# google-research/simclr

Hardware: AMD Instinct MI355X
Metric: images/sec (whole node), ResNet-50 1x SimCLR pretraining step @224px (higher is better)
Workload: dtype f32; 1 GPU; ResNet-50 1x, 224x224, 2 views/image, per-GPU batch 512, global batch 512, NT-Xent T=0.1 + linear-eval head + LARS, global BN, dp1; global_batch=512, parallelism=dp1

## Files before the change

simclr_amd/csrc/conv.hip:

```cpp
#include "common.h"
#include <stdlib.h>
#include <string.h>
#include <mutex>
#include <type_traits>

namespace {

enum { MODE_FWD = 0, MODE_DGRAD = 1 };

struct ConvP {
  const void* x;
  const void* w;
  void* y;
  float* stats;
  int V, IH, IW, IC, OH, OW, N, KH, KW, stride, pad;
  int pixpitch;
  int M, K;
  int nslot, accumulate;
  int m_tiles, n_tiles;
  int cs, py, px, cls_h, cls_w;
  int ntaps;
  int taps[9];
  unsigned long long tap_w, dy_w, dx_w;
  const void* bn_x;
// ... 1919 lines not shown
    const unsigned char* ds = xs + p.hpp * RB;
#pragma unroll
    for (int ks = 0; ks < 2; ++ks) {
      u32x4 bf[4];
#pragma unroll
      for (int ni = 0; ni < 4; ++ni) {
        const s16x4_t lo = __builtin_amdgcn_ds_read_tr16_b64_v4i16((lds_s16x4_t*)(ds + ks * 32 * RB + b_lo[ni]));
        const s16x4_t hi = __builtin_amdgcn_ds_read_tr16_b64_v4i16((lds_s16x4_t*)(ds + ks * 32 * RB + b_hi[ni]));
        const u32x2 l2 = __builtin_bit_cast(u32x2, lo), h2 = __builtin_bit_cast(u32x2, hi);
        bf[ni] = (u32x4){l2[0], l2[1], h2[0], h2[1]};
      }
      const int jw = p.W - gx[ks];
      const unsigned lowm = jw >= 8 ? 0xffu : ((1u << jw) - 1u);
      const int y1 = (gy[ks] + 1 == p.H) ? 0 : gy[ks] + 1;
      const unsigned up = (gy[ks] > 0 ? lowm : 0u) | (y1 > 0 ? (0xffu & ~lowm) : 0u);
      const unsigned dn = (gy[ks] < p.H - 1 ? lowm : 0u) | (y1 < p.H - 1 ? (0xffu & ~lowm) : 0u);
      const unsigned lf = 0xffu & ~((gx[ks] == 0 ? 1u : 0u) | (jw < 8 ? (1u << jw) : 0u));
      const unsigned rt = 0xffu & ~((jw - 1 < 8 ? (1u << (jw - 1)) : 0u) |
                                    (jw - 1 + p.W < 8 ? (1u << (jw - 1 + p.W)) : 0u));
      u32x4 wup, wdn, wlf, wrt;
#pragma unroll
      for (int d = 0; d < 4; ++d) {
        wup[d] = (((up >> (2 * d)) & 1u) ? 0x0000ffffu : 0u) | (((up >> (2 * d + 1)) & 1u) ? 0xffff0000u : 0u);
        wdn[d] = (((dn >> (2 * d)) & 1u) ? 0x0000ffffu : 0u) | (((dn >> (2 * d + 1)) & 1u) ? 0xffff0000u : 0u);
        wlf[d] = (((lf >> (2 * d)) & 1u) ? 0x0000ffffu : 0u) | (((lf >> (2 * d + 1)) & 1u) ? 0xffff0000u : 0u);
        wrt[d] = (((rt >> (2 * d)) & 1u) ? 0x0000ffffu : 0u) | (((rt >> (2 * d + 1)) & 1u) ? 0xffff0000u : 0u);
      }
#pragma unroll
      for (int t = 0; t < 9; ++t) {
        const int ty = t / 3, tx = t % 3;
        const s16x4_t lo = __builtin_amdgcn_ds_read_tr16_b64_v4i16((lds_s16x4_t*)(xs + ks * 32 * RB + a_lo[t]));
        const s16x4_t hi = __builtin_amdgcn_ds_read_tr16_b64_v4i16((lds_s16x4_t*)(xs + ks * 32 * RB + a_hi[t]));
        const u32x2 l2 = __builtin_bit_cast(u32x2, lo), h2 = __builtin_bit_cast(u32x2, hi);
        u32x4 af = (u32x4){l2[0], l2[1], h2[0], h2[1]};
        if (t != 4) {
#pragma unroll
          for (int d = 0; d < 4; ++d) {
            unsigned w = 0xffffffffu;
            if (ty == 0) w &= wup[d]; else if (ty == 2) w &= wdn[d];
            if (tx == 0) w &= wlf[d]; else if (tx == 2) w &= wrt[d];
            af[d] &= w;
          }
        }
#pragma unroll
        for (int ni = 0; ni < 4; ++ni)
          acc[t][ni] = __builtin_amdgcn_mfma_f32_16x16x32_bf16(
              __builtin_bit_cast(bf16x8, bf[ni]), __builtin_bit_cast(bf16x8, af), acc[t][ni], 0, 0, 0);
      }
      gx[ks] += dcol;
      if (gx[ks] >= p.W) { gx[ks] -= p.W; ++gy[ks]; }
      gy[ks] += drow;
      if (gy[ks] >= p.H) gy[ks] -= p.H;
    }
  };

  int issued = c_begin, cs = 0, is = ST - 1;
#pragma unroll
  for (int s = 0; s < ST - 1; ++s)
    if (issued < c_end) { issue(issued, s); ++issued; }
  const int nq = p.hpp >> 5;
  for (int c = c_begin; c < c_end; ++c) {
    if (ST == 3 && issued - c - 1 >= 1 && nq == 3) asm volatile("s_waitcnt vmcnt(5)" ::: "memory");
    else if (ST == 3 && issued - c - 1 >= 1 && nq == 4) asm volatile("s_waitcnt vmcnt(6)" ::: "memory");
    else asm volatile("s_waitcnt vmcnt(0)" ::: "memory");
    __syncthreads();
    if (issued < c_end) { issue(issued, is); ++issued; is = (is + 1 == ST) ? 0 : is + 1; }
    compute(cs);
    cs = (cs + 1 == ST) ? 0 : cs + 1;
  }
  float* slab = p.dw + (long long)split * 9 * p.IC * p.N;
#pragma unroll
  for (int t = 0; t < 9; ++t) {
    const int kk = t * p.IC + ci0 + wave * 16 + fl;
#pragma unroll
    for (int ni = 0; ni < 4; ++ni) {
      const int n = n0 + ni * 16 + g * 4;
      *(float4*)(slab + (long long)kk * p.N + n) = make_float4(acc[t][ni][0], acc[t][ni][1], acc[t][ni][2], acc[t][ni][3]);
    }
  }
}

__device__ __forceinline__ int w3f_key(int row) { return (row & 3) | (((row >> 3) & 1) << 2); }

__global__ __launch_bounds__(256, 2) void conv_wgrad3x3_f32ps(const Wgrad3P p) {
  constexpr int BR = 32, RB = 256;
  extern __shared__ __attribute__((aligned(16))) unsigned char smem[];
  typedef __attribute__((address_space(1))) const void* gptr_t;
  typedef __attribute__((address_space(3))) void* lptr_t;
  const int tid = threadIdx.x, lane = tid & 63;
  const int wave = __builtin_amdgcn_readfirstlane(tid >> 6);
  const int g = lane >> 4, fl = lane & 15;
  const int tiles = p.ci_tiles * p.co_tiles;
  const int xcd = blockIdx.x & 7, bidx = blockIdx.x >> 3;
  const int tile = bidx % tiles, split = (bidx / tiles) * 8 + xcd;
  if (split >= p.splits) return;
  const int ci0 = (tile % p.ci_tiles) * 64, n0 = (tile / p.ci_tiles) * 64;
  const float* __restrict__ X = (const float*)p.x;
  const float* __restrict__ DY = (const float*)p.dy;
  const int W1 = p.W + 1;
  const int stage_bytes = (p.hpp + BR) * RB;

  f32x4 acc[9][4];
#pragma unroll
  for (int t = 0; t < 9; ++t)
#pragma unroll
    for (int j = 0; j < 4; ++j) acc[t][j] = (f32x4){0.f, 0.f, 0.f, 0.f};

  const int nchunks = (p.M + BR - 1) / BR;
  const int c_begin = split * p.chunks_per_split;
  const int c_end = min(nchunks, c_begin + p.chunks_per_split);

  const int lrow = lane >> 4, lpc = lane & 15;
  auto issue = [&](int c, int s) __attribute__((always_inline)) {
    unsigned char* xs = smem + s * stage_bytes;
    unsigned char* ds = xs + p.hpp * RB;
    const int mc = c * BR;
    const int nxi = p.hpp >> 2;
    for (int q = wave; q < nxi; q += 4) {
      const int r = q * 4 + lrow;
      const int lc = (((lpc >> 1) ^ w3f_key(r)) << 1) | (lpc & 1);
      const int gp = mc + r - W1;
      const void* src = (gp >= 0 && gp < p.M) ? (const void*)(X + (long long)gp * p.pixpitch + ci0 + lc * 4) : p.zero;
      __builtin_amdgcn_global_load_lds((gptr_t)src, (lptr_t)(xs + q * 1024), 16, 0, 0);
    }
#pragma unroll
    for (int j = 0; j < 2; ++j) {
      const int q = wave * 2 + j;
      const int r = q * 4 + lrow;
      const int lc = (((lpc >> 1) ^ w3f_key(r)) << 1) | (lpc & 1);
      const int m = mc + r;
      const void* src = (m < p.M) ? (const void*)(DY + (long long)m * p.N + n0 + lc * 4) : p.zero;
      __builtin_amdgcn_global_load_lds((gptr_t)src, (lptr_t)(ds + q * 1024), 16, 0, 0);
    }
  };

  auto off_of = [&](int row, int byte) -> int { return row * RB + (((byte >> 5) ^ w3f_key(row)) << 5) + (byte & 31); };
  const int px_lane = g * 8 + (fl >> 2);
  const int xbyte = (wave >> 1) * 128 + (wave & 1) * 32 + (fl & 3) * 8;
  auto hi_of = [](int o) __attribute__((always_inline)) -> int { return ((o & ~7) + 4 * RB) ^ ((o & 1) << 7); };
  int a_lo[9];
#pragma unroll
  for (int t = 0; t < 9; ++t) {
    const int r = px_lane + W1 + (t / 3 - 1) * p.W + (t % 3 - 1);
    a_lo[t] = off_of(r, xbyte) | ((r >> 2) & 1);
  }
  int b_lo[4];
#pragma unroll
  for (int ni = 0; ni < 4; ++ni) {
    const int nbyte = (ni >> 1) * 128 + (ni & 1) * 32 + (fl & 3) * 8;
    b_lo[ni] = off_of(px_lane, nbyte) | ((px_lane >> 2) & 1);
  }
  auto frag = [&](const unsigned char* base, int o_lo, int o_hi) __attribute__((always_inline)) -> u32x4 {
    const s16x4_t lo = __builtin_amdgcn_ds_read_tr16_b64_v4i16((lds_s16x4_t*)(base + o_lo));
    const s16x4_t hi = __builtin_amdgcn_ds_read_tr16_b64_v4i16((lds_s16x4_t*)(base + o_hi));
    const u32x2 l2 = __builtin_bit_cast(u32x2, lo), h2 = __builtin_bit_cast(u32x2, hi);
    return (u32x4){l2[0], l2[1], h2[0], h2[1]};
  };

  const int hw = p.H * p.W;
  const int dq = BR / hw, drem = BR - dq * hw, drow = drem / p.W, dcol = drem - drow * p.W;
  int gy, gx;
  {
    const int m = c_begin * BR + g * 8;
    const int rem = m % hw;
    gy = rem / p.W; gx = rem - gy * p.W;
  }

  auto convert = [&](int s) __attribute__((always_inline)) {
    unsigned char* xs = smem + s * stage_bytes;
    for (int q = tid; q < p.hpp * 8; q += 256) {
      const int row = q >> 3, j = (q >> 2) & 1, gq = q & 3;
      u32x4* w0 = (u32x4*)(xs + off_of(row, (j * 8 + gq) * 16));
      u32x4* w1 = (u32x4*)(xs + off_of(row, (j * 8 + 4 + gq) * 16));
      u32x4 hi, lo;
      split_terms2(*w0, *w1, hi, lo);
      *w0 = hi; *w1 = lo;
    }
  };

  auto compute = [&](int s) __attribute__((always_inline)) {
    const unsigned char* xs = smem + s * stage_bytes;
    const unsigned char* ds = xs + p.hpp * RB;
    u32x4 dh[4], dl[4];
#pragma unroll
    for (int ni = 0; ni < 4; ++ni) {
      const int o0 = b_lo[ni] & ~7, o1 = hi_of(b_lo[ni]);
      dh[ni] = frag(ds, o0, o1);
      dl[ni] = frag(ds, o0 ^ 64, o1 ^ 64);
    }
    const int jw = p.W - gx;
    const unsigned lowm = jw >= 8 ? 0xffu : ((1u << jw) - 1u);
    const int y1 = (gy + 1 == p.H) ? 0 : gy + 1;
    const unsigned up = (gy > 0 ? lowm : 0u) | (y1 > 0 ? (0xffu & ~lowm) : 0u);
    const unsigned dn = (gy < p.H - 1 ? lowm : 0u) | (y1 < p.H - 1 ? (0xffu & ~lowm) : 0u);
    const unsigned lf = 0xffu & ~((gx == 0 ? 1u : 0u) | (jw < 8 ? (1u << jw) : 0u));
    const unsigned rt = 0xffu & ~((jw - 1 < 8 ? (1u << (jw - 1)) : 0u) | (jw - 1 + p.W < 8 ? (1u << (jw - 1 + p.W)) : 0u));
    __builtin_amdgcn_s_setprio(1);
#pragma unroll
    for (int t = 0; t < 9; ++t) {
      const int ty = t / 3, tx = t % 3;
      const int o0 = a_lo[t] & ~7, o1 = hi_of(a_lo[t]);
      u32x4 xh = frag(xs, o0, o1);
      u32x4 xl = frag(xs, o0 ^ 64, o1 ^ 64);
      if (t != 4) {
        const unsigned m8 = (ty == 0 ? up : ty == 2 ? dn : 0xffu) & (tx == 0 ? lf : tx == 2 ? rt : 0xffu);
#pragma unroll
        for (int d = 0; d < 4; ++d) {
          const unsigned w = ((unsigned)__builtin_amdgcn_sbfe((int)m8, 2 * d, 1) & 0x0000ffffu) |
                             ((unsigned)__builtin_amdgcn_sbfe((int)m8, 2 * d + 1, 1) & 0xffff0000u);
          xh[d] &= w; xl[d] &= w;
        }
      }
#pragma unroll
      for (int ni = 0; ni < 4; ++ni) acc[t][ni] = mma_bf16(dl[ni], xh, acc[t][ni]);
#pragma unroll
      for (int ni = 0; ni < 4; ++ni) acc[t][ni] = mma_bf16(dh[ni], xl, acc[t][ni]);
#pragma unroll
      for (int ni = 0; ni < 4; ++ni) acc[t][ni] = mma_bf16(dh[ni], xh, acc[t][ni]);
      __builtin_amdgcn_sched_barrier(0);
    }
    __builtin_amdgcn_s_setprio(0);
    gx += dcol;
    if (gx >= p.W) { gx -= p.W; ++gy; }
    gy += drow;
    if (gy >= p.H) gy -= p.H;
  };

  int issued = c_begin, cs = 0, is = 1;
  if (issued < c_end) { issue(issued, 0); ++issued; }
  for (int c = c_begin; c < c_end; ++c) {
    asm volatile("s_waitcnt vmcnt(0)" ::: "memory");
    __syncthreads();
    if (issued < c_end) { issue(issued, is); ++issued; is ^= 1; }
    convert(cs);
    __syncthreads();
    compute(cs);
    cs ^= 1;
  }
  float* slab = p.dw + (long long)split * 9 * p.IC * p.N;
  const int Qx = 4 * (wave & 1) + (fl >> 2);
  const int ci = ci0 + (wave >> 1) * 32 + (Qx & 1) * 16 + (Qx >> 1) * 4 + (fl & 3);
#pragma unroll
  for (int t = 0; t < 9; ++t) {
    const int kk = t * p.IC + ci;
#pragma unroll
    for (int ni = 0; ni < 4; ++ni) {
      const int Q = 4 * (ni & 1) + g;
      const int n = n0 + (ni >> 1) * 32 + (Q & 1) * 16 + (Q >> 1) * 4;
      *(float4*)(slab + (long long)kk * p.N + n) = make_float4(acc[t][ni][0], acc[t][ni][1], acc[t][ni][2], acc[t][ni][3]);
    }
  }
}

template <int TT>
__global__ __launch_bounds__(256) void small_gemm_nt_f32(const float* __restrict__ A, const float* __restrict__ B,
                                                         float* __restrict__ C, int M, int N, int K) {
  constexpr int LDR = 36;
  constexpr int FR = TT / 32;
  constexpr int LPT = TT * 8 / 256;
  __shared__ __attribute__((aligned(16))) float As[TT * LDR], Bs[TT * LDR];
  const int tid = threadIdx.x, lane = tid & 63, wave = tid >> 6;
  const int fl = lane & 15, q = lane >> 4;
  const int wm = wave >> 1, wn = wave & 1;
  const int m0 = blockIdx.y * TT, n0 = blockIdx.x * TT;
  f32x4 acc[FR][FR];
#pragma unroll
  for (int i = 0; i < FR; ++i)
#pragma unroll
    for (int j = 0; j < FR; ++j) acc[i][j] = (f32x4){0.f, 0.f, 0.f, 0.f};
  float4 ra[LPT], rb[LPT];
  auto gload = [&](int k0) __attribute__((always_inline)) {
#pragma unroll
    for (int l = 0; l < LPT; ++l) {
      const int idx = tid + l * 256, r = idx >> 3, c = (idx & 7) * 4;
      ra[l] = (m0 + r < M) ? *(const float4*)(A + (long long)(m0 + r) * K + k0 + c) : make_float4(0.f, 0.f, 0.f, 0.f);
      rb[l] = (n0 + r < N) ? *(const float4*)(B + (long long)(n0 + r) * K + k0 + c) : make_float4(0.f, 0.f, 0.f, 0.f);
    }
  };
  gload(0);
  for (int k0 = 0; k0 < K; k0 += 32) {
    __syncthreads();
#pragma unroll
    for (int l = 0; l < LPT; ++l) {
      const int idx = tid + l * 256, r = idx >> 3, c = (idx & 7) * 4;
      *(float4*)(As + r * LDR + c) = ra[l];
      *(float4*)(Bs + r * LDR + c) = rb[l];
    }
    __syncthreads();
    if (k0 + 32 < K) gload(k0 + 32);
#pragma unroll
    for (int h = 0; h < 2; ++h) {
      float4 af[FR], bf[FR];
#pragma unroll
      for (int i = 0; i < FR; ++i) {
        af[i] = *(const float4*)(As + (wm * (FR * 16) + i * 16 + fl) * LDR + h * 16 + 4 * q);
        bf[i] = *(const float4*)(Bs + (wn * (FR * 16) + i * 16 + fl) * LDR + h * 16 + 4 * q);
      }
#pragma unroll
      for (int i = 0; i < FR; ++i)
#pragma unroll
        for (int j = 0; j < FR; ++j) {
          acc[i][j] = __builtin_amdgcn_mfma_f32_16x16x4f32(bf[j].x, af[i].x, acc[i][j], 0, 0, 0);
          acc[i][j] = __builtin_amdgcn_mfma_f32_16x16x4f32(bf[j].y, af[i].y, acc[i][j], 0, 0, 0);
          acc[i][j] = __builtin_amdgcn_mfma_f32_16x16x4f32(bf[j].z, af[i].z, acc[i][j], 0, 0, 0);
          acc[i][j] = __builtin_amdgcn_mfma_f32_16x16x4f32(bf[j].w, af[i].w, acc[i][j], 0, 0, 0);
        }
    }
  }
#pragma unroll
  for (int i = 0; i < FR; ++i) {
    const int m = m0 + wm * (FR * 16) + i * 16 + fl;
#pragma unroll
    for (int j = 0; j < FR; ++j) {
      const int n = n0 + wn * (FR * 16) + j * 16 + q * 4;
      if (m < M && n < N) *(float4*)(C + (long long)m * N + n) = make_float4(acc[i][j][0], acc[i][j][1], acc[i][j][2], acc[i][j][3]);
    }
  }
}

__global__ __launch_bounds__(256) void slab_reduce(const float* __restrict__ slabs, int splits, long long numel,
// ... 590 lines not shown
static bool dry_run() { return simclr_dry_run(); }
template <typename T, int MODE> static void record_inst(const char* kern, unsigned grid, unsigned block, size_t lds, const ConvP& p) {
  snprintf(g_last_inst, sizeof(g_last_inst), "(%s) elt=%d role=%s grid=%u block=%u lds=%zu m_tiles=%d n_tiles=%d tail_parts=%d", kern,
           (int)sizeof(T), MODE == MODE_FWD ? "fwd" : "dgrad", grid, block, lds, p.m_tiles, p.n_tiles, p.rem_parts);
}
template <typename T> static const char* type_name() { return sizeof(T) == 2 ? "uint16_t" : "float"; }
static const char* mode_name(int mode) { return mode == MODE_FWD ? "MODE_FWD" : "MODE_DGRAD"; }
static const char* tf(bool v) { return v ? "true" : "false"; }

template <typename T, int MODE, int BN, bool STATS, bool GLDS>
static void run_igemm(dim3 grid, dim3 block, size_t lds, hipStream_t stream, const ConvP& p) {
  char name[128];
  snprintf(name, sizeof(name), "conv_igemm<%s, %s, %d, %s, %s>", type_name<T>(), mode_name(MODE), BN, tf(STATS), tf(GLDS));
  record_inst<T, MODE>(name, grid.x, block.x, lds, p);
  if (!dry_run()) hipLaunchKernelGGL((conv_igemm<T, MODE, BN, STATS, GLDS>), grid, block, lds, stream, p);
}

template <int MODE, bool STATS, bool BNEPI, bool FLAT>
static void run_wide(dim3 grid, dim3 block, size_t lds, hipStream_t stream, const ConvP& p) {
  char name[128];
  snprintf(name, sizeof(name), "conv_igemm_wide<%s, %s, %s, %s>", mode_name(MODE), tf(STATS), tf(BNEPI), tf(FLAT));
  record_inst<uint16_t, MODE>(name, grid.x, block.x, lds, p);
  if (!dry_run()) hipLaunchKernelGGL((conv_igemm_wide<MODE, STATS, BNEPI, FLAT>), grid, block, lds, stream, p);
}

template <typename T, int MODE, int BM, int BN, int NW, int STAGES, bool STATS, bool BNEPI, bool EXT = false,
          bool WIN = false, bool FAPPLY = false, int SPL = 0, bool TAIL = false, bool PSB = false, int FAS = 0, int EPS = 0, bool PSX = false>
static void run_persistent(dim3 grid, dim3 block, size_t lds, hipStream_t stream, const ConvP& p) {
  const int opt[9] = {EXT, WIN, FAPPLY, SPL, TAIL, PSB, FAS, EPS, PSX};
  const bool is_bool[9] = {true, true, true, false, true, true, false, false, true};
  int n = 9;
  while (n > 0 && opt[n - 1] == 0) --n;
  char name[256];
  int len = snprintf(name, sizeof(name), "conv_igemm_persistent<%s, %s, %d, %d, %d, %d, %s, %s", type_name<T>(), mode_name(MODE), BM, BN, NW,
                     STAGES, tf(STATS), tf(BNEPI));
  for (int i = 0; i < n; ++i)
    len += is_bool[i] ? snprintf(name + len, sizeof(name) - len, ", %s", tf(opt[i])) : snprintf(name + len, sizeof(name) - len, ", %d", opt[i]);
  snprintf(name + len, sizeof(name) - len, ">");
  record_inst<T, MODE>(name, grid.x, block.x, lds, p);
  if (!dry_run())
    hipLaunchKernelGGL((conv_igemm_persistent<T, MODE, BM, BN, NW, STAGES, STATS, BNEPI, EXT, WIN, FAPPLY, SPL, TAIL, PSB, FAS, EPS, PSX>),
                       grid, block, lds, stream, p);
}

struct WgradRec { int k_tiles, n_tiles, splits, chunks_per_split, xcd_map; };
static WgradRec rec_of(const WgradP& p) { return {p.k_tiles, p.n_tiles, p.splits, p.chunks_per_split, p.xcd_map}; }
static WgradRec rec_of(const Wgrad3P& p) { return {p.ci_tiles, p.co_tiles, p.splits, p.chunks_per_split, 1}; }
static WgradRec rec_of(const StemWgP& p) { return {1, 1, p.splits, p.chunks_per_split, 0}; }
static void record_wgrad(const char* kern, int elt, const char* role, unsigned grid, unsigned block, size_t lds, const WgradRec& r) {
  snprintf(g_last_inst, sizeof(g_last_inst), "(%s) elt=%d role=%s grid=%u block=%u lds=%zu k_tiles=%d n_tiles=%d splits=%d chunks_per_split=%d xcd_map=%d",
           kern, elt, role, grid, block, lds, r.k_tiles, r.n_tiles, r.splits, r.chunks_per_split, r.xcd_map);
}

template <typename T, int BKW, int BNW, bool MT = false>
static void run_wgrad(const char* role, unsigned grid, unsigned block, size_t lds, hipStream_t stream, const WgradP& p) {
  char name[128];
  snprintf(name, sizeof(name), MT ? "conv_wgrad<%s, %d, %d, true>" : "conv_wgrad<%s, %d, %d>", type_name<T>(), BKW, BNW);
  record_wgrad(name, (int)sizeof(T), role, grid, block, lds, rec_of(p));
  if (!dry_run()) hipLaunchKernelGGL((conv_wgrad<T, BKW, BNW, MT>), dim3(grid), dim3(block), lds, stream, p);
}

template <typename T, int BKW, int BNW, int BRM, int STAGES, int WK = 2, int WNN = 2, bool GRAM = false, bool MT = false, int SPL = 0, int PSD = 0>
static void run_wgrad_dma(const char* role, unsigned grid, unsigned block, size_t lds, hipStream_t stream, const WgradP& p) {
  const int opt[6] = {WK, WNN, GRAM, MT, SPL, PSD}, dflt[6] = {2, 2, 0, 0, 0, 0};
  const bool is_bool[6] = {false, false, true, true, false, false};
  int n = 6;
  while (n > 0 && opt[n - 1] == dflt[n - 1]) --n;
  char name[160];
  int len = snprintf(name, sizeof(name), "conv_wgrad_dma<%s, %d, %d, %d, %d", type_name<T>(), BKW, BNW, BRM, STAGES);
  for (int i = 0; i < n; ++i)
    len += is_bool[i] ? snprintf(name + len, sizeof(name) - len, ", %s", tf(opt[i])) : snprintf(name + len, sizeof(name) - len, ", %d", opt[i]);
  snprintf(name + len, sizeof(name) - len, ">");
  record_wgrad(name, (int)sizeof(T), role, grid, block, lds, rec_of(p));
  if (!dry_run())
    hipLaunchKernelGGL((conv_wgrad_dma<T, BKW, BNW, BRM, STAGES, WK, WNN, GRAM, MT, SPL, PSD>), dim3(grid), dim3(block), lds, stream, p);
}

template <int ST> static void run_wgrad3x3_bf16(unsigned grid, unsigned block, size_t lds, hipStream_t stream, const Wgrad3P& q) {
  char name[64];
  snprintf(name, sizeof(name), "conv_wgrad3x3_bf16<%d>", ST);
  record_wgrad(name, 2, "wgrad", grid, block, lds, rec_of(q));
  if (!dry_run()) hipLaunchKernelGGL(conv_wgrad3x3_bf16<ST>, dim3(grid), dim3(block), lds, stream, q);
}
static void run_wgrad3x3_f32ps(unsigned grid, unsigned block, size_t lds, hipStream_t stream, const Wgrad3P& q) {
  record_wgrad("conv_wgrad3x3_f32ps", 4, "wgrad", grid, block, lds, rec_of(q));
  if (!dry_run()) hipLaunchKernelGGL(conv_wgrad3x3_f32ps, dim3(grid), dim3(block), lds, stream, q);
}
template <int STAGES> static void run_stem_wgrad_ps(unsigned grid, unsigned block, size_t lds, hipStream_t stream, const StemWgP& p) {
  char name[64];
  snprintf(name, sizeof(name), "stem_wgrad_ps<7, 2, %d>", STAGES);
  record_wgrad(name, 4, "stem_wgrad_ps", grid, block, lds, rec_of(p));
  if (!dry_run()) hipLaunchKernelGGL((stem_wgrad_ps<7, 2, STAGES>), dim3(grid), dim3(block), lds, stream, p);
}
static void run_slab_reduce(const void* slabs, int splits, long long numel, float* out, int accumulate, hipStream_t stream) {
  const int grid = max(1, (int)ceil_div(numel / 4, 16));
  const size_t len = strlen(g_last_inst);
  snprintf(g_last_inst + len, sizeof(g_last_inst) - len, " reduce_grid=%d", grid);
  if (!dry_run()) hipLaunchKernelGGL(slab_reduce, dim3(grid), dim3(256), 0, stream, (const float*)slabs, splits, numel, out, accumulate);
}

static const void* zero_page() {
  static void* zp = nullptr;
  if (dry_run()) return (const void*)&g_last_inst;
  if (!zp && hipGetSymbolAddress(&zp, HIP_SYMBOL(g_zero16)) != hipSuccess) zp = nullptr;
  return zp;
}

static void igemm_persistent_grid(long long M, int N, int* bn, int* n_tiles, int* grid, bool narrow = false) {
  const int BN = (N <= 64 || narrow) ? 64 : 128;
  const int m_tiles = (int)((M + 127) / 128);
  const int nt = ceil_div(N, BN);
  const int unit = 8 * nt;
  const int resident = (BN == 64 ? 3 : 2) * 256;
  int pg = (resident / unit) * unit;
  if (pg < unit) pg = unit;
  const int need = ceil_div(m_tiles, 8) * unit;
  if (pg > need) pg = need;
  *bn = BN; *n_tiles = nt; *grid = pg;
}

static bool igemm_use_256(const ConvP& p, bool fwd) {
  if (p.N % 256 != 0 || p.ntaps <= 0 || p.N / 256 > 32) return false;
  const char* e = getenv("SIMCLR_IGEMM_TILE");
  const int mode = e ? atoi(e) : 0;
  if (mode == 256) return true;
  if (mode == 128) return false;
  if (p.KH != 1 || p.KW != 1 || p.M < 150000) return false;
  if (p.bn_mode && !p.fapply) return false;
  if (fwd && !p.fapply && p.stats && p.K < 128) return false;
  return !p.fapply;
}

static bool igemm_use_wide(const ConvP& p, bool fwd) {
  const char* e = getenv("SIMCLR_IGEMM_WIDE");
  const int mode = e ? atoi(e) : 1;
  if (mode == 0) return false;
  if (p.N % 256 != 0 || p.N / 256 > 32 || p.ntaps <= 0 || p.IC % 64 != 0 || p.x2 || p.fapply) return false;
  if (p.bn_mode && p.bn_mode != 4 && !p.bn_x) return false;
  if ((long long)p.V * p.IH * p.IW * p.pixpitch * 2 >= 0xE0000000ll || (long long)p.N * p.K * 2 >= 0xE0000000ll) return false;
  if (mode == 2) return true;
  if (p.M < 32768) return false;
  if (fwd) return !(p.KH == 3 && p.KW == 3 && p.stride == 1) && 2.0 * (double)p.M * p.K * p.N >= 3.0e11;
  return !p.bn_mode && !p.accumulate && p.KH == 1 && p.KW == 1 && p.IC >= 512;
}

static bool igemm_narrow(const ConvP& p, size_t esz, bool dgrad = false) {
  constexpr int kmax = 64;
  constexpr int kmax32 = 128;
  if (esz == 4)
    return dgrad && p.split == 3 && p.N > 64 && p.KH == 1 && p.KW == 1 && p.stride == 1 && !p.x2 && p.K <= kmax32 && p.N / 64 <= 64;
  return esz == 2 && p.N > 64 && p.KH == 1 && p.KW == 1 && p.stride == 1 && !p.x2 && p.K <= kmax && p.N / 64 <= 64;
}

static std::mutex g_scratch_mutex;

struct SplitScratch { hipStream_t stream; float* ws; size_t floats; unsigned* flags; size_t nflags; };
static SplitScratch g_split_scratch[8];
static int g_split_scratch_n = 0;

static thread_local int g_last_split_parts = 0;
static void split_tail_plan(ConvP& p, int grid, int units, int unit_steps, bool wide = false) {
  p.rem_parts = 0; p.rem_full = 0; p.rem_tiles = 0; p.part_ws = nullptr; p.part_flags = nullptr; p.part_err = nullptr;
  const char* e = getenv("SIMCLR_IGEMM_SPLIT");
  const int mode = e ? atoi(e) : (wide ? 1 : 0);
  if (mode == 0 || p.n_tiles <= 0 || grid % p.n_tiles != 0) return;
  const int mslots = grid / p.n_tiles;
  const int full = p.m_tiles / mslots, R = p.m_tiles - full * mslots;
  const int max_parts = mode > 1 ? mode : 8;
  int P = R > 0 ? mslots / R : 0;
// ... 355 lines not shown
          }
      q.M = p.V * q.cls_h * q.cls_w;
      if (q.ntaps == 0 && p.accumulate == 2 && ((py | px) & 1)) q.accumulate = 0;
      else if (q.ntaps == 0 && p.accumulate) continue;
      if (p.accumulate == 3) q.accumulate = 0;
      if (q.ntaps == 0) q.x_ps = 0;
      if (plan_igemm<T, MODE>(q, true, true).family == IgemmPlan::UNSUPPORTED) return 1;
      cls[n++] = q;
    }
  for (int i = 0; i < n; ++i)
    if (int rc = launch_igemm_one<T, MODE>(cls[i], stream)) return rc;
  return 0;
}

struct ConvCall { int dtype, terms; bool w_ps, x_ps; };
static int conv_call(const char* fn, int dtype, bool fwd, int ps_w_terms, bool ps_in, int Cout, ConvCall* c) {
  c->terms = terms_of(&dtype, fwd);
  SIMCLR_CHECK_ARG(c->terms >= 0, "%s: bad matrix-arithmetic field in dtype (SIMCLR_FMT_TERMS)", fn);
  c->w_ps = ps_w_terms && take_ps_w(&dtype);
  SIMCLR_CHECK_ARG(!c->w_ps || ((dtype & 0xff) == SIMCLR_DT_F32 && c->terms == ps_w_terms),
                   "%s: pre-split weights (SIMCLR_FMT_PS_W) need fp32 storage and terms %d", fn, ps_w_terms);
  c->x_ps = ps_in && (dtype & SIMCLR_FMT_PS_IN) != 0;
  if (ps_in) dtype &= 0xff;
  SIMCLR_CHECK_ARG(!c->x_ps || (dtype == SIMCLR_DT_F32 && c->terms == 3 && Cout % 32 == 0),
                   "%s: a pre-split dy needs fp32 storage, three backward terms (simclr_set_f32_matmul) and Cout %% 32 == 0", fn);
  c->dtype = dtype;
  return 0;
}
static int conv_params(const ConvCall& c, const void* x, const void* w, void* y, int V, int IH, int IW, int IC, int OH, int OW, int N,
                       int KH, int KW, int stride, int pad, ConvP* p) {
  *p = {};
  p->zero = zero_page();
  SIMCLR_CHECK_ARG(p->zero != nullptr, "conv2d: zero page symbol not found");
  p->w_ps = c.w_ps ? 1 : 0; p->x_ps = c.x_ps ? 1 : 0;
  p->split = c.terms;
  p->x = x; p->w = w; p->y = y;
  p->V = V; p->IH = IH; p->IW = IW; p->IC = IC; p->OH = OH; p->OW = OW; p->N = N;
  p->KH = KH; p->KW = KW; p->stride = stride; p->pad = pad; p->pixpitch = IC;
  p->M = V * OH * OW; p->K = KH * KW * IC;
  return 0;
}
template <int MODE> static int launch_conv(int dtype, const ConvP& p, hipStream_t stream) {
  return dtype == SIMCLR_DT_BF16 ? launch_igemm<uint16_t, MODE>(p, stream) : launch_igemm<float, MODE>(p, stream);
}


static int env_int(const char* name, int dflt) { const char* e = getenv(name); return e ? atoi(e) : dflt; }

static int wgrad_splits(long long M, int K, int N, int bkw, int bnw, int br, int* chunks_per_split, int cap, int target) {
  const int tiles = ceil_div(K, bkw) * ceil_div(N, bnw);
  const int nchunks = ceil_div(M, br);
  int splits = max(1, min(nchunks, target / max(1, tiles)));
  if (nchunks >= 8) splits = min(nchunks / 8 * 8, max(8, (splits + 7) / 8 * 8));
  splits = min(splits, cap);
  *chunks_per_split = ceil_div(nchunks, splits);
  int eff = ceil_div(nchunks, *chunks_per_split);
  while (nchunks >= 8 && eff % 8 != 0 && *chunks_per_split > 1) {
    --*chunks_per_split;
    eff = ceil_div(nchunks, *chunks_per_split);
    if (eff > cap) { ++*chunks_per_split; eff = ceil_div(nchunks, *chunks_per_split); break; }
  }
  return eff;
}

struct WgradShape { int V, IH, IW, Cin, pixpitch, OH, OW, Cout, KH, KW, stride, pad; };
struct WgradPlan {
  enum Family {
    UNSUPPORTED,
    NINE_TAP_BF16,
    NINE_TAP_F32PS,
    TILE256_BF16,
    TILE256_F32,
    STEM_DMA_BF16,
    STEM_DMA_F32,
    STEM_MT,
    REG_STAGED,
    DMA_RING,
    GRAM,
    STEM_PS
  } family;
  int bkw, bnw;
  int stages, br;
  int hpp;
  int splits, chunks_per_split;
  int k_tiles, n_tiles, xcd_map;
  unsigned grid, block;
  size_t lds;
};

static bool wgrad_takes_presplit(const WgradShape& s, int dtype, int terms) {
  return dtype == SIMCLR_DT_F32 && terms == 3 && s.Cin % 64 == 0 && s.Cout % 32 == 0 && (s.pixpitch * 4) % 16 == 0;
}

static WgradPlan plan_wgrad(const WgradShape& s, int dtype, int terms, bool dy_ps) {
  WgradPlan k = {};
  const bool bf = dtype == SIMCLR_DT_BF16;
  const int esz = bf ? 2 : 4, taps = s.KH * s.KW, K = taps * s.Cin, N = s.Cout;
  const long long M = (long long)s.V * s.OH * s.OW;
  const bool aligned = (s.pixpitch * esz) % 16 == 0;
  k.block = 256;
  if (env_int("SIMCLR_WGRAD_3X3", 1) > 0 && s.KH == 3 && s.KW == 3 && s.stride == 1 && s.pad == 1 && s.IH == s.OH && s.IW == s.OW &&
      s.Cin % 64 == 0 && s.Cout % 64 == 0 && s.IW >= 7 && (bf ? aligned : (terms == 3 && dy_ps))) {
    const int br = bf ? 64 : 32;
    const int hpp = (br + 2 * s.IW + 2 + 31) / 32 * 32;
    const size_t stage = (size_t)(hpp + br) * 64 * esz;
    if ((bf ? 2 : 4) * stage <= 160 * 1024) {
      k.family = bf ? WgradPlan::NINE_TAP_BF16 : WgradPlan::NINE_TAP_F32PS;
      k.bkw = 64; k.bnw = 64; k.br = br; k.hpp = hpp;
      k.stages = (bf && 2 * 3 * stage <= 160 * 1024) ? 3 : 2;
      k.k_tiles = s.Cin / 64; k.n_tiles = N / 64;
      const int tiles = k.k_tiles * k.n_tiles;
      const int want = min(bf ? 4096 : 2048, max(8, env_int("SIMCLR_WGRAD3_BLOCKS", tiles == 1 ? 2048 : 512)));
      k.splits = wgrad_splits(M, s.Cin, N, 64, 64, br, &k.chunks_per_split, 2048, want);
      k.xcd_map = 1;
      k.grid = tiles * ceil_div(k.splits, 8) * 8;
      k.lds = k.stages * stage;
      return k;
    }
  }
  k.bkw = (s.Cin % 128 == 0) ? 128 : (s.Cin % 64 == 0 ? 64 : 32);
  k.bnw = (N % 128 == 0 || N > 128) ? 128 : 64;
  if (k.bkw == 32) k.bnw = 64;
  if (s.Cin % 256 == 0 && N % 256 == 0 && aligned) {
    if (bf && env_int("SIMCLR_WGRAD_256", 1) != 0 && (M >= 500000 || (taps == 9 && M >= 150000 && s.Cin == 256))) k.bkw = k.bnw = 256;
    if (!bf && terms == 3 && dy_ps && s.stride == 1 && taps == 1) k.bkw = k.bnw = 256;
  }
  const bool stem = k.bkw == 32 && s.Cin == 32 && K <= 256 && N <= 64;
  if (stem) { k.bkw = 256; k.bnw = 64; }
  int cfg = env_int("SIMCLR_WGRAD_CFG", -1);
  if (cfg < 0 || (!bf && cfg > 1)) cfg = 1;
  if (k.bkw == 32 || stem || !aligned) cfg = 0;
  const bool big = k.bkw == 128 && k.bnw == 128, big256 = k.bkw == 256 && !stem;
  if (big256 && cfg == 0) cfg = 1;
  if (dy_ps && cfg == 0) return k;
  const int brm = ((cfg >= 2 && big) || (big256 && bf)) ? 1 : 2;
  k.stages = big256 ? (bf ? 4 : 2) : (cfg <= 1 ? 2 : (big ? (cfg == 2 ? 3 : 4) : 3));
  k.br = (bf ? 32 : 16) * brm;
  const int target = stem ? 1024 : (k.bkw == 256 ? 512 : env_int("SIMCLR_WGRAD_BLOCKS", bf ? 1024 : 1536));
  k.splits = wgrad_splits(M, K, N, k.bkw, k.bnw, k.br, &k.chunks_per_split, stem ? 1024 : 256, target);
  k.k_tiles = ceil_div(K, k.bkw);
  k.n_tiles = ceil_div(N, k.bnw);
  k.xcd_map = cfg != 0 || M >= 1500000 || (M >= 500000 && taps == 1 && s.stride == 1);
#ifdef SIMCLR_DIAG
  { const char* e = getenv("SIMCLR_WGRAD_XCD"); if (e && atoi(e) >= 0) k.xcd_map = atoi(e); }
#endif
  k.family = big256 ? (bf ? WgradPlan::TILE256_BF16 : WgradPlan::TILE256_F32) : cfg == 0 ? WgradPlan::REG_STAGED : WgradPlan::DMA_RING;
  if (big256) k.block = 512;
  if (stem) {
    const bool packed = s.KW == 1 && s.pad == 0 && s.pixpitch == 4;
    k.family = WgradPlan::STEM_MT;
    if (bf && packed && s.stride % 2 == 0 && s.IW % 2 == 0) {
      k.family = WgradPlan::STEM_DMA_BF16;
    } else if (!bf && packed && terms != 0 && env_int("SIMCLR_STEM_SPLIT", 1) != 0) {
      k.family = WgradPlan::STEM_DMA_F32;
      k.block = 512;
      if (terms == 3 && env_int("SIMCLR_STEM_WGRAD_STAGES", 2) == 3) k.stages = 3;
    }
    if (k.family != WgradPlan::STEM_MT) k.xcd_map = 1;
  }
  k.grid = k.k_tiles * k.n_tiles * (k.xcd_map ? ceil_div(k.splits, 8) * 8 : k.splits);
  k.lds = (size_t)k.stages * k.br * (k.bkw + k.bnw) * esz;
  return k;
}

static WgradPlan plan_gram(long long M, int K, int dtype) {
  WgradPlan k = {};
  const bool bf = dtype == SIMCLR_DT_BF16;
  k.family = WgradPlan::GRAM;
  k.bkw = k.bnw = K;
  k.stages = 4;
  k.br = (bf ? 64 : 32) / (K == 256 ? 2 : 1);
  const int ranges = K == 256 ? 512 : 1024;
  k.splits = wgrad_splits(M, K, K, K, K, k.br, &k.chunks_per_split, ranges, ranges);
  k.k_tiles = 1; k.n_tiles = 1; k.xcd_map = 1;
  k.grid = ceil_div(k.splits, 8) * 8;
  k.block = K == 256 ? 512 : 256;
  k.lds = (size_t)k.stages * k.br * K * (bf ? 2 : 4);
  return k;
}

static WgradPlan plan_stem_wgrad_ps(int V, int OH, int OW) {
  WgradPlan k = {};
  k.family = WgradPlan::STEM_PS;
  k.bkw = 7 * 32; k.bnw = 64; k.br = 32;
  const long long chunks = (long long)V * OH * ((OW + 31) / 32);
  const int want = (int)max(1ll, min((long long)max(8, min(env_int("SIMCLR_STEM_WGRAD_BLOCKS", 1024), 1024)), chunks));
  k.chunks_per_split = (int)((chunks + want - 1) / want);
  k.splits = (int)((chunks + k.chunks_per_split - 1) / k.chunks_per_split);
  k.stages = env_int("SIMCLR_STEM_WGRAD_PS_STAGES", 2) == 3 ? 3 : 2;
  k.k_tiles = 1; k.n_tiles = 1;
  k.grid = k.splits; k.block = 128;
  k.lds = (size_t)k.stages * ((7 * 70 + 63) / 64 + 8) * 1024;
  return k;
}

template <int A, int B> struct WgradTile { static constexpr int BKW = A, BNW = B; };
template <typename F> static void with_wgrad_tile(int bkw, int bnw, F&& f) {
  if (bkw == 128 && bnw == 128) f(WgradTile<128, 128>());
  else if (bkw == 128) f(WgradTile<128, 64>());
// ... 206 lines not shown
  ConvCall c;
  if (int rc = conv_call("conv2d_dgrad_bn_ext", dtype, false, 0, false, Cout, &c)) return rc;
  dtype = c.dtype;
  const int epc = dtype == SIMCLR_DT_BF16 ? 8 : 4;
  SIMCLR_CHECK_ARG(dtype == SIMCLR_DT_BF16 || dtype == SIMCLR_DT_F32, "conv2d_dgrad_bn_ext: bad dtype %d", dtype);
  SIMCLR_CHECK_ARG(Cout % (8 * epc) == 0 && Cin % (8 * epc) == 0, "conv2d_dgrad_bn_ext: Cin=%d / Cout=%d must be multiples of %d", Cin, Cout, 8 * epc);
  SIMCLR_CHECK_ARG((long long)V * H * W < (1ll << 31), "conv2d_dgrad_bn_ext: M overflows int32");
  SIMCLR_CHECK_ARG(mask_mode >= 1 && mask_mode <= 4, "conv2d_dgrad_bn_ext: mask_mode must be 1, 2, 3 or 4");
  SIMCLR_CHECK_ARG(dm && h && w_ext && stats && nslot > 0 && (mask_mode == 4 || (bn_x && bn_mean && bn_rstd)), "conv2d_dgrad_bn_ext: null argument");
  SIMCLR_CHECK_ARG(mask_mode == 2 || bn_mask, "conv2d_dgrad_bn_ext: mask_mode 1 / 3 / 4 need bn_mask");
  SIMCLR_CHECK_ARG(mask_mode != 2 || (bn_scale && bn_shift), "conv2d_dgrad_bn_ext: mask_mode 2 needs scale/shift");
  ConvP p;
  if (int rc = conv_params(c, dm, w_ext, dx, V, H, W, Cout, H, W, Cin, 1, 1, 1, 0, &p)) return rc;
  p.stats = stats; p.nslot = nslot; p.accumulate = accumulate;
  p.K = Cout + Cin;
  p.x2 = h; p.ic2 = Cin; p.pixpitch2 = Cin; p.bias = bias;
  p.bn_x = bn_x; p.bn_mask = bn_mask; p.bn_scale = bn_scale; p.bn_shift = bn_shift;
  p.bn_mean = bn_mean; p.bn_rstd = bn_rstd; p.bn_mode = mask_mode;
  SIMCLR_CHECK_ARG(launch_conv<MODE_DGRAD>(dtype, p, stream) == 0, "conv2d_dgrad_bn_ext: no kernel for this launch");
  SIMCLR_CHECK_LAUNCH();
  return 0;
}

int simclr_conv2d_dgrad_ext(const void* dm, const void* h, const void* w_ext, const float* bias, void* dx, int accumulate,
                            int V, int H, int W, int Cin, int Cout, int dtype, hipStream_t stream) {
  ConvCall c;
  if (int rc = conv_call("conv2d_dgrad_ext", dtype, false, 0, false, Cout, &c)) return rc;
  dtype = c.dtype;
  const int epc = dtype == SIMCLR_DT_BF16 ? 8 : 4;
  SIMCLR_CHECK_ARG(dtype == SIMCLR_DT_BF16 || dtype == SIMCLR_DT_F32, "conv2d_dgrad_ext: bad dtype %d", dtype);
  SIMCLR_CHECK_ARG(Cout % (8 * epc) == 0 && Cin % (8 * epc) == 0, "conv2d_dgrad_ext: Cin=%d / Cout=%d must be multiples of %d", Cin, Cout, 8 * epc);
  SIMCLR_CHECK_ARG((long long)V * H * W < (1ll << 31), "conv2d_dgrad_ext: M overflows int32");
  SIMCLR_CHECK_ARG(dm && h && w_ext && dx, "conv2d_dgrad_ext: null argument");
  ConvP p;
  if (int rc = conv_params(c, dm, w_ext, dx, V, H, W, Cout, H, W, Cin, 1, 1, 1, 0, &p)) return rc;
  p.nslot = 1; p.accumulate = accumulate;
  p.K = Cout + Cin;
  p.x2 = h; p.ic2 = Cin; p.pixpitch2 = Cin; p.bias = bias;
  SIMCLR_CHECK_ARG(launch_conv<MODE_DGRAD>(dtype, p, stream) == 0, "conv2d_dgrad_ext: no kernel for this launch");
  SIMCLR_CHECK_LAUNCH();
  return 0;
}

size_t simclr_conv2d_wgrad_workspace_bytes(int V, int OH, int OW, int Cin, int Cout, int KH, int KW, int dtype) {
  int splits = 0;
  for (int stride = 1; stride <= 2; ++stride)
    for (int odd_pitch = 0; odd_pitch <= 1; ++odd_pitch) {
      const WgradShape s = {V, OH * stride, OW * stride, Cin, Cin + odd_pitch, OH, OW, Cout, KH, KW, stride, (KH - 1) / 2};
      for (int terms : {0, 3, 6})
        for (int ps = 0; ps <= 1; ++ps) {
          if (dtype == SIMCLR_DT_BF16 ? (terms != 0 || ps) : (!valid_terms(terms, false) || (ps && !wgrad_takes_presplit(s, dtype, terms)))) continue;
          const WgradPlan k = plan_wgrad(s, dtype, terms, ps != 0);
          if (k.family != WgradPlan::UNSUPPORTED) splits = max(splits, k.splits);
        }
    }
  return (size_t)splits * KH * KW * Cin * Cout * sizeof(float);
}

int simclr_conv2d_wgrad(const void* x, const void* dy, float* dw, int accumulate, void* workspace,
                        int V, int IH, int IW, int Cin, int pixpitch, int OH, int OW, int Cout, int KH,
                        int KW, int stride, int pad, int dtype, hipStream_t stream) {
  const int terms = terms_of(&dtype, false);
  SIMCLR_CHECK_ARG(terms >= 0, "conv2d_wgrad: bad matrix-arithmetic field in dtype (SIMCLR_FMT_TERMS)");
  const bool dy_ps = (dtype & SIMCLR_FMT_PS_IN) != 0;
  dtype &= 0xff;
  const WgradShape s = {V, IH, IW, Cin, pixpitch, OH, OW, Cout, KH, KW, stride, pad};
  SIMCLR_CHECK_ARG(!dy_ps || wgrad_takes_presplit(s, dtype, terms),
                   "conv2d_wgrad: a pre-split dy needs fp32 storage, three backward terms, Cin %% 64 == 0 and Cout %% 32 == 0 (Cin=%d Cout=%d)", Cin, Cout);
  SIMCLR_CHECK_ARG(dtype == SIMCLR_DT_BF16 || dtype == SIMCLR_DT_F32, "conv2d_wgrad: bad dtype %d", dtype);
  SIMCLR_CHECK_ARG(Cin % 32 == 0, "conv2d_wgrad: Cin=%d must be a multiple of 32", Cin);
  SIMCLR_CHECK_ARG(Cout % 8 == 0, "conv2d_wgrad: Cout=%d must be a multiple of 8", Cout);
  SIMCLR_CHECK_ARG((long long)V * OH * OW < (1ll << 31), "conv2d_wgrad: M overflows int32");
  const WgradPlan k = plan_wgrad(s, dtype, terms, dy_ps);
  SIMCLR_CHECK_ARG(k.family != WgradPlan::UNSUPPORTED, "conv2d_wgrad: no pre-split kernel on the register-staged path");
  const void* zero = zero_page();
  SIMCLR_CHECK_ARG(zero != nullptr, "conv2d_wgrad: zero page symbol not found");
  const int M = V * OH * OW, K = KH * KW * Cin;
  if (k.family == WgradPlan::NINE_TAP_BF16 || k.family == WgradPlan::NINE_TAP_F32PS) {
    Wgrad3P q = {};
    q.x = x; q.dy = dy; q.dw = (float*)workspace; q.zero = zero;
    q.V = V; q.H = IH; q.W = IW; q.IC = Cin; q.N = Cout; q.pixpitch = pixpitch; q.M = M;
    q.ci_tiles = k.k_tiles; q.co_tiles = k.n_tiles;
    q.splits = k.splits; q.chunks_per_split = k.chunks_per_split; q.hpp = k.hpp;
    if (k.family == WgradPlan::NINE_TAP_F32PS) run_wgrad3x3_f32ps(k.grid, k.block, k.lds, stream, q);
    else if (k.stages == 3) run_wgrad3x3_bf16<3>(k.grid, k.block, k.lds, stream, q);
    else run_wgrad3x3_bf16<2>(k.grid, k.block, k.lds, stream, q);
  } else {
    WgradP p = {};
    p.x = x; p.dy = dy; p.dw = (float*)workspace; p.zero = zero;
    p.V = V; p.IH = IH; p.IW = IW; p.IC = Cin; p.OH = OH; p.OW = OW; p.N = Cout;
    p.KH = KH; p.KW = KW; p.stride = stride; p.pad = pad; p.pixpitch = pixpitch;
    p.M = M; p.K = K;
    p.splits = k.splits; p.chunks_per_split = k.chunks_per_split;
    p.k_tiles = k.k_tiles; p.n_tiles = k.n_tiles; p.xcd_map = k.xcd_map;
    p.split = terms;
    p.dy_ps = dy_ps ? 1 : 0;
#ifdef SIMCLR_DIAG
    { const char* e = getenv("SIMCLR_DIAG"); p.diag = e ? atoi(e) : 0; }
#endif
    launch_wgrad(k, dtype == SIMCLR_DT_BF16, stream, p);
  }
  SIMCLR_CHECK_LAUNCH();
  run_slab_reduce(workspace, k.splits, (long long)K * Cout, dw, accumulate, stream);
  SIMCLR_CHECK_LAUNCH();
  return 0;
}

size_t simclr_conv2d_gram_workspace_bytes(long long M, int K, int dtype) {
  return (size_t)plan_gram(M, K, dtype).splits * ((size_t)K * K + K) * sizeof(float);
}
int simclr_conv2d_gram(const void* h, float* out, void* workspace, long long M, int K, int dtype, hipStream_t stream) {
  const int terms = terms_of(&dtype, true);
  SIMCLR_CHECK_ARG(terms >= 0, "conv2d_gram: bad matrix-arithmetic field in dtype (SIMCLR_FMT_TERMS)");
  SIMCLR_CHECK_ARG(dtype == SIMCLR_DT_BF16 || dtype == SIMCLR_DT_F32, "conv2d_gram: bad dtype %d", dtype);
  SIMCLR_CHECK_ARG(K == 64 || K == 128 || (K == 256 && dtype == SIMCLR_DT_BF16), "conv2d_gram: K=%d not supported (64, 128, bf16 256)", K);
  SIMCLR_CHECK_ARG(M > 0 && M < (1ll << 31), "conv2d_gram: bad M");
  const WgradPlan k = plan_gram(M, K, dtype);
  WgradP p = {};
  p.x = h; p.dy = h; p.dw = (float*)workspace;
  p.V = 1; p.IH = 1; p.IW = (int)M; p.IC = K; p.OH = 1; p.OW = (int)M; p.N = K;
  p.KH = 1; p.KW = 1; p.stride = 1; p.pad = 0; p.pixpitch = K;
  p.M = (int)M; p.K = K;
  p.splits = k.splits; p.chunks_per_split = k.chunks_per_split;
  p.k_tiles = k.k_tiles; p.n_tiles = k.n_tiles; p.xcd_map = k.xcd_map;
  p.zero = zero_page();
  SIMCLR_CHECK_ARG(p.zero != nullptr, "conv2d_gram: zero page symbol not found");
  if (K == 256) run_wgrad_dma<uint16_t, 256, 256, 1, 4, 2, 4, true>("gram", k.grid, k.block, k.lds, stream, p);
  else if (dtype == SIMCLR_DT_BF16) {
    if (K == 64) run_wgrad_dma<uint16_t, 64, 64, 2, 4, 2, 2, true>("gram", k.grid, k.block, k.lds, stream, p);
    else run_wgrad_dma<uint16_t, 128, 128, 2, 4, 2, 2, true>("gram", k.grid, k.block, k.lds, stream, p);
  } else if (terms != 0) {
    if (K == 64) run_wgrad_dma<float, 64, 64, 2, 4, 2, 2, true, false, 6>("gram", k.grid, k.block, k.lds, stream, p);
    else run_wgrad_dma<float, 128, 128, 2, 4, 2, 2, true, false, 6>("gram", k.grid, k.block, k.lds, stream, p);
  } else {
    if (K == 64) run_wgrad_dma<float, 64, 64, 2, 4, 2, 2, true>("gram", k.grid, k.block, k.lds, stream, p);
    else run_wgrad_dma<float, 128, 128, 2, 4, 2, 2, true>("gram", k.grid, k.block, k.lds, stream, p);
  }
  SIMCLR_CHECK_LAUNCH();
  run_slab_reduce(workspace, k.splits, (long long)K * K + K, out, 0, stream);
  SIMCLR_CHECK_LAUNCH();
  return 0;
}

int simclr_small_gemm_nt_f32(const float* A, const float* B, float* C, int M, int N, int K, hipStream_t stream) {
  SIMCLR_CHECK_ARG(M > 0 && N > 0 && K > 0 && M % 16 == 0 && N % 16 == 0 && K % 32 == 0, "small_gemm_nt_f32: M=%d N=%d must be multiples of 16, K=%d of 32", M, N, K);
  if ((long long)ceil_div(M, 64) * ceil_div(N, 64) >= 256)
    hipLaunchKernelGGL((small_gemm_nt_f32<64>), dim3(ceil_div(N, 64), ceil_div(M, 64)), dim3(256), 0, stream, A, B, C, M, N, K);
  else
    hipLaunchKernelGGL((small_gemm_nt_f32<32>), dim3(ceil_div(N, 32), ceil_div(M, 32)), dim3(256), 0, stream, A, B, C, M, N, K);
  SIMCLR_CHECK_LAUNCH();
  return 0;
}

int simclr_stem_conv_fwd(const void* xp, const void* w_s, void* y, float* stats, int nslot, int V,
                         int HP, int WP, int OH, int OW, int Cout, int KHP, int KWP, int stride,
                         int dtype, hipStream_t stream) {
  const int terms = terms_of(&dtype, true);
  SIMCLR_CHECK_ARG(terms >= 0, "stem_conv_fwd: bad matrix-arithmetic field in dtype (SIMCLR_FMT_TERMS)");
  SIMCLR_CHECK_ARG(dtype == SIMCLR_DT_BF16 || dtype == SIMCLR_DT_F32, "stem_conv_fwd: bad dtype %d", dtype);
  const int epc = dtype == SIMCLR_DT_BF16 ? 8 : 4;
  StemP p = {};
  p.xp = xp; p.w = w_s; p.y = y; p.stats = stats; p.nslot = nslot > 0 ? nslot : 1;
  p.V = V; p.HP = HP; p.WP = WP; p.OH = OH; p.OW = OW; p.N = Cout; p.KHP = KHP; p.KWP = KWP;
  p.stride = stride; p.M = V * OH * OW; p.KP = KHP * KWP * 4;
  SIMCLR_CHECK_ARG(p.KP % (4 * epc) == 0, "stem_conv_fwd: padded K=%d not a multiple of %d", p.KP, 4 * epc);
  SIMCLR_CHECK_ARG((KWP * 4) % epc == 0, "stem_conv_fwd: KWP*4 must be a multiple of %d", epc);
  SIMCLR_CHECK_ARG(Cout % (dtype == SIMCLR_DT_BF16 ? 8 : 4) == 0, "stem_conv_fwd: Cout=%d must be a multiple of %d", Cout, dtype == SIMCLR_DT_BF16 ? 8 : 4);
// ... 137 lines not shown
```

Before: 3793 images/s.

## Add ring-buffered halo variant of fp32 3x3 wgrad kernel for larger images

Adds a RING template variant of the fp32 pre-split 3x3 weight-gradient kernel. Input halo rows live in a 192-row circular LDS buffer, so each chunk loads and converts only the BR new rows instead of the whole halo tile. This lets shapes whose double-buffered stage would exceed LDS (hpp==160, the 56x56 layers) use the nine-tap kernel instead of the generic wgrad path. It also halves the default block count for those shapes. It adds modular offset arithmetic and a single-buffered halo, which serialises halo loads against compute.

Result: no change. 3830 images/s, median of 6 (+1.0%).

```diff
diff --git a/simclr_amd/csrc/conv.hip b/simclr_amd/csrc/conv.hip
--- a/simclr_amd/csrc/conv.hip
+++ b/simclr_amd/csrc/conv.hip
@@ -2025,7 +2025,9 @@
 
 __device__ __forceinline__ int w3f_key(int row) { return (row & 3) | (((row >> 3) & 1) << 2); }
 
+template <bool RING>
 __global__ __launch_bounds__(256, 2) void conv_wgrad3x3_f32ps(const Wgrad3P p) {
+  constexpr int RR = 192;
   constexpr int BR = 32, RB = 256;
   extern __shared__ __attribute__((aligned(16))) unsigned char smem[];
   typedef __attribute__((address_space(1))) const void* gptr_t;
@@ -2121,9 +2123,7 @@
     }
   };
 
-  auto compute = [&](int s) __attribute__((always_inline)) {
-    const unsigned char* xs = smem + s * stage_bytes;
-    const unsigned char* ds = xs + p.hpp * RB;
+  auto compute_at = [&](const unsigned char* xs, const unsigned char* ds) __attribute__((always_inline)) {
     u32x4 dh[4], dl[4];
 #pragma unroll
     for (int ni = 0; ni < 4; ++ni) {
@@ -2142,7 +2142,9 @@
 #pragma unroll
     for (int t = 0; t < 9; ++t) {
       const int ty = t / 3, tx = t % 3;
-      const int o0 = a_lo[t] & ~7, o1 = hi_of(a_lo[t]);
+      const int o0 = a_lo[t] & ~7;
+      int o1 = hi_of(a_lo[t]);
+      if (RING && o1 >= RR * RB) o1 -= RR * RB;
       u32x4 xh = frag(xs, o0, o1);
       u32x4 xl = frag(xs, o0 ^ 64, o1 ^ 64);
       if (t != 4) {
@@ -2168,17 +2170,75 @@
     gy += drow;
     if (gy >= p.H) gy -= p.H;
   };
-
-  int issued = c_begin, cs = 0, is = 1;
-  if (issued < c_end) { issue(issued, 0); ++issued; }
-  for (int c = c_begin; c < c_end; ++c) {
-    asm volatile("s_waitcnt vmcnt(0)" ::: "memory");
-    __syncthreads();
-    if (issued < c_end) { issue(issued, is); ++issued; is ^= 1; }
-    convert(cs);
-    __syncthreads();
-    compute(cs);
-    cs ^= 1;
+  auto compute = [&](int s) __attribute__((always_inline)) { compute_at(smem + s * stage_bytes, smem + s * stage_bytes + p.hpp * RB); };
+
+  if constexpr (RING) {
+    unsigned char* dsb = smem + RR * RB;
+    auto issue_rows = [&](int c, int r0, int r1, int rot) __attribute__((always_inline)) {
+      const int mc = c * BR;
+      for (int q = (r0 >> 2) + wave; q < (r1 >> 2); q += 4) {
+        const int r = q * 4 + lrow;
+        int pq = q + (rot >> 2);
+        if (pq >= RR / 4) pq -= RR / 4;
+        const int lc = (((lpc >> 1) ^ w3f_key(r)) << 1) | (lpc & 1);
+        const int gp = mc + r - W1;
+        const void* src = (gp >= 0 && gp < p.M) ? (const void*)(X + (long long)gp * p.pixpitch + ci0 + lc * 4) : p.zero;
+        __builtin_amdgcn_global_load_lds((gptr_t)src, (lptr_t)(smem + pq * 1024), 16, 0, 0);
+      }
+    };
+    auto issue_dy = [&](int c, unsigned char* ds) __attribute__((always_inline)) {
+      const int mc = c * BR;
+#pragma unroll
+      for (int j = 0; j < 2; ++j) {
+        const int q = wave * 2 + j;
+        const int r = q * 4 + lrow;
+        const int lc = (((lpc >> 1) ^ w3f_key(r)) << 1) | (lpc & 1);
+        const int m = mc + r;
+        const void* src = (m < p.M) ? (const void*)(DY + (long long)m * p.N + n0 + lc * 4) : p.zero;
+        __builtin_amdgcn_global_load_lds((gptr_t)src, (lptr_t)(ds + q * 1024), 16, 0, 0);
+      }
+    };
+    auto convert_rows = [&](int r0, int r1, int rot) __attribute__((always_inline)) {
+      for (int q = r0 * 8 + tid; q < r1 * 8; q += 256) {
+        int row = (q >> 3) + rot;
+        if (row >= RR) row -= RR;
+        const int j = (q >> 2) & 1, gq = q & 3;
+        u32x4* w0 = (u32x4*)(smem + off_of(row, (j * 8 + gq) * 16));
+        u32x4* w1 = (u32x4*)(smem + off_of(row, (j * 8 + 4 + gq) * 16));
+        u32x4 hi, lo;
+        split_terms2(*w0, *w1, hi, lo);
+        *w0 = hi; *w1 = lo;
+      }
+    };
+    int rot = 0, cur = 0;
+    if (c_begin < c_end) { issue_rows(c_begin, 0, p.hpp, 0); issue_dy(c_begin, dsb); }
+    for (int c = c_begin; c < c_end; ++c) {
+      asm volatile("s_waitcnt vmcnt(0)" ::: "memory");
+      __syncthreads();
+      const int nrot = rot + BR >= RR ? rot + BR - RR : rot + BR;
+      if (c + 1 < c_end) { issue_rows(c + 1, p.hpp - BR, p.hpp, nrot); issue_dy(c + 1, dsb + (cur ^ 1) * BR * RB); }
+      convert_rows(c == c_begin ? 0 : p.hpp - BR, p.hpp, rot);
+      __syncthreads();
+      compute_at(smem, dsb + cur * BR * RB);
+#pragma unroll
+      for (int t = 0; t < 9; ++t) {
+        a_lo[t] += BR * RB;
+        if (a_lo[t] >= RR * RB) a_lo[t] -= RR * RB;
+      }
+      rot = nrot; cur ^= 1;
+    }
+  } else {
+    int issued = c_begin, cs = 0, is = 1;
+    if (issued < c_end) { issue(issued, 0); ++issued; }
+    for (int c = c_begin; c < c_end; ++c) {
+      asm volatile("s_waitcnt vmcnt(0)" ::: "memory");
+      __syncthreads();
+      if (issued < c_end) { issue(issued, is); ++issued; is ^= 1; }
+      convert(cs);
+      __syncthreads();
+      compute(cs);
+      cs ^= 1;
+    }
   }
   float* slab = p.dw + (long long)split * 9 * p.IC * p.N;
   const int Qx = 4 * (wave & 1) + (fl >> 2);
@@ -2935,9 +2995,9 @@
   record_wgrad(name, 2, "wgrad", grid, block, lds, rec_of(q));
   if (!dry_run()) hipLaunchKernelGGL(conv_wgrad3x3_bf16<ST>, dim3(grid), dim3(block), lds, stream, q);
 }
-static void run_wgrad3x3_f32ps(unsigned grid, unsigned block, size_t lds, hipStream_t stream, const Wgrad3P& q) {
-  record_wgrad("conv_wgrad3x3_f32ps", 4, "wgrad", grid, block, lds, rec_of(q));
-  if (!dry_run()) hipLaunchKernelGGL(conv_wgrad3x3_f32ps, dim3(grid), dim3(block), lds, stream, q);
+template <bool RING> static void run_wgrad3x3_f32ps(unsigned grid, unsigned block, size_t lds, hipStream_t stream, const Wgrad3P& q) {
+  record_wgrad(RING ? "conv_wgrad3x3_f32ps<true>" : "conv_wgrad3x3_f32ps<false>", 4, "wgrad", grid, block, lds, rec_of(q));
+  if (!dry_run()) hipLaunchKernelGGL(conv_wgrad3x3_f32ps<RING>, dim3(grid), dim3(block), lds, stream, q);
 }
 template <int STAGES> static void run_stem_wgrad_ps(unsigned grid, unsigned block, size_t lds, hipStream_t stream, const StemWgP& p) {
   char name[64];
@@ -3459,6 +3519,7 @@
   int bkw, bnw;
   int stages, br;
   int hpp;
+  bool ring;
   int splits, chunks_per_split;
   int k_tiles, n_tiles, xcd_map;
   unsigned grid, block;
@@ -3481,17 +3542,18 @@
     const int br = bf ? 64 : 32;
     const int hpp = (br + 2 * s.IW + 2 + 31) / 32 * 32;
     const size_t stage = (size_t)(hpp + br) * 64 * esz;
-    if ((bf ? 2 : 4) * stage <= 160 * 1024) {
+    const bool ring = !bf && 4 * stage > 160 * 1024 && hpp == 160;
+    if ((bf ? 2 : 4) * stage <= 160 * 1024 || ring) {
       k.family = bf ? WgradPlan::NINE_TAP_BF16 : WgradPlan::NINE_TAP_F32PS;
-      k.bkw = 64; k.bnw = 64; k.br = br; k.hpp = hpp;
+      k.bkw = 64; k.bnw = 64; k.br = br; k.hpp = hpp; k.ring = ring;
       k.stages = (bf && 2 * 3 * stage <= 160 * 1024) ? 3 : 2;
       k.k_tiles = s.Cin / 64; k.n_tiles = N / 64;
       const int tiles = k.k_tiles * k.n_tiles;
-      const int want = min(bf ? 4096 : 2048, max(8, env_int("SIMCLR_WGRAD3_BLOCKS", tiles == 1 ? 2048 : 512)));
+      const int want = min(bf ? 4096 : 2048, max(8, env_int("SIMCLR_WGRAD3_BLOCKS", tiles == 1 ? (ring ? 1024 : 2048) : 512)));
       k.splits = wgrad_splits(M, s.Cin, N, 64, 64, br, &k.chunks_per_split, 2048, want);
       k.xcd_map = 1;
       k.grid = tiles * ceil_div(k.splits, 8) * 8;
-      k.lds = k.stages * stage;
+      k.lds = ring ? (size_t)(192 + 2 * br) * 64 * esz : k.stages * stage;
       return k;
     }
   }
@@ -3864,7 +3926,8 @@
     q.V = V; q.H = IH; q.W = IW; q.IC = Cin; q.N = Cout; q.pixpitch = pixpitch; q.M = M;
     q.ci_tiles = k.k_tiles; q.co_tiles = k.n_tiles;
     q.splits = k.splits; q.chunks_per_split = k.chunks_per_split; q.hpp = k.hpp;
-    if (k.family == WgradPlan::NINE_TAP_F32PS) run_wgrad3x3_f32ps(k.grid, k.block, k.lds, stream, q);
+    if (k.family == WgradPlan::NINE_TAP_F32PS && k.ring) run_wgrad3x3_f32ps<true>(k.grid, k.block, k.lds, stream, q);
+    else if (k.family == WgradPlan::NINE_TAP_F32PS) run_wgrad3x3_f32ps<false>(k.grid, k.block, k.lds, stream, q);
     else if (k.stages == 3) run_wgrad3x3_bf16<3>(k.grid, k.block, k.lds, stream, q);
     else run_wgrad3x3_bf16<2>(k.grid, k.block, k.lds, stream, q);
   } else {
```
